# zju-vipa/ProtoPFormer

Measured on AMD Instinct MI355X. Metric: images/sec train step, deit_small+2000 protos, bs256, 1/2/4/8 MI355X, higher is better.
Workload: dtype bf16; 1 GPU; deit_small_patch16_224, synthetic 224x224, 2000x384 prototypes, 200 classes, k=81, batch 256/GPU (BASELINE.json configs[2]), train step = fwd+CE+PPC+bwd+allreduce+AdamW+EMA, DropPath 0.1; blocks after the token reservation run compacted on the 1+k reserved rows (equal to the masked full-length blocks to bf16 rounding); bf16 backbone: the reserved tokens differ from the fp32 reference's in ~2-3 % o; global_batch=256, parallelism=dp1

## Files before the change

### include/ppf_hip.h

```cpp
#ifndef PPF_HIP_H
#define PPF_HIP_H

#include <stddef.h>
#include <stdint.h>

#ifdef __cplusplus
extern "C" {
#endif

typedef struct ihipStream_t* ppf_stream_t;

#define PPF_ERR_SHAPE (-1)
#define PPF_ERR_ALIGN (-2)
#define PPF_ERR_ARG (-3)

#define PPF_ABI_VERSION 10

const char* ppf_last_error(void);
int ppf_abi_version(void);
int ppf_device_info(int* cu_count, int* clock_mhz, char* name, int name_len);
int ppf_stream_arm(ppf_stream_t stream, int on);
int ppf_stream_wait_stream(ppf_stream_t dst, ppf_stream_t src);
int64_t ppf_stream_mark(ppf_stream_t stream);
int ppf_stream_wait_mark(ppf_stream_t stream, int64_t ticket);
// ... 157 lines not shown
                        ppf_stream_t stream);
int ppf_assemble_tokens_bwd(const float* dx, void* dtok, float* dpos, float* dcls, int B, int Np, int D, int lead,
                            ppf_stream_t stream);
int ppf_sigmoid_bwd_blocks(int rows);
int ppf_sigmoid_bwd(const float* df, const float* f, void* dz, float* dbias, int rows, int cols, float* partial, size_t partial_bytes,
                    ppf_stream_t stream);
int ppf_adamw_step(float* p, const float* g, float* m, float* v, float* ema, void* p16, int64_t n, int nseg,
                   const int64_t* seg_bounds, const float* seg_lr, const float* seg_wd, float beta1, float beta2, float eps,
                   int step, float ema_decay, float grad_scale, ppf_stream_t stream);
int ppf_adamw_step_dev(float* p, const float* g, float* m, float* v, float* ema, void* p16, int64_t n, int nseg,
                       const int64_t* seg_bounds, const float* hyper, float beta1, float beta2, float eps, float ema_decay,
                       ppf_stream_t stream);
int ppf_adamw_step_guarded(float* p, const float* g, float* m, float* v, float* ema, void* p16, int64_t n, int nseg,
                           const int64_t* seg_bounds, const float* hyper, float beta1, float beta2, float eps, float ema_decay,
                           const float* loss, int* nonfinite_flag, ppf_stream_t stream);
int ppf_hyper_set(float* hyper, const float* host_vals, int n, ppf_stream_t stream);
int ppf_clip_grad_blocks(void);
int ppf_clip_grad_scale(const float* g, int64_t n, float max_norm, float pre_scale, float* partial, float* hyper, float* norm_out,
                        ppf_stream_t stream);
int ppf_droppath_scales(float* out, const float* keep, int nslot, int B, uint64_t seed, void* state_u64, ppf_stream_t stream);
int ppf_reserved_rows_map(const int* idx, int* rows, int B, int k, int N, ppf_stream_t stream);
int ppf_gather_rows(const void* src, const int* rows, void* dst, int nrows, int row_bytes, ppf_stream_t stream);
int ppf_scatter_rows(const void* src, const int* rows, void* dst, int nrows_src, int nrows_dst, int row_bytes, ppf_stream_t stream);
int ppf_memset_zero(void* ptr, size_t bytes, ppf_stream_t stream);
int ppf_copy_2d(void* dst, int64_t dst_pitch, const void* src, int64_t src_pitch, int64_t width, int64_t rows, ppf_stream_t stream);
int ppf_image_finish_u8(const void* in_u8_hwc, float* out_nchw, int B, int H, int W, const float* mean3, const float* std3,
                        const int* rects, uint64_t seed, const void* state_u64, ppf_stream_t stream);
#define PPF_MIX_KIND 0
#define PPF_MIX_YL 1
#define PPF_MIX_YH 2
// ... 27 lines not shown
```

### protopformer_amd/backbone.py

```python
import functools
import os

import torch
import torch.nn as nn

from . import _lib, ops
from .ops import EPI_ATOMIC, EPI_BF16, EPI_DGELU, EPI_F32, EPI_GELU, EPI_RESID, EPI_SIGMOID_F32

LN_EPS = 1e-6
_KEEP_CACHE = {}
_ROW_BWD_MAX_ELEMS = 12_000_000


def _row_bwd(M, D):
    return M * D <= _ROW_BWD_MAX_ELEMS


def droppath_scales(rates, B, device, training):
    slots = [r if training else 0.0 for r in rates]
    active = [i for i, r in enumerate(slots) if r > 0.0]
    if not active:
        return None, [-1] * len(slots)
    key = (tuple(slots), str(device))
    st = _KEEP_CACHE.get(key)
# ... 167 lines not shown
        d = ops.ew_bwd_f32(5, ops.linear_dgrad_f32(d, c.weight), x_in)
    ops.colsum_f32(d, gv(convs[0].bias))
    return ops.cast_bf16(d)


class WgradLane:

    def __init__(self, device):
        self.enabled = os.environ.get("PPF_WGRAD_STREAM", "1") != "0"
        self.streams = [torch.cuda.Stream(device=device)] if self.enabled else []
        self.raws = [st.cuda_stream for st in self.streams]
        self.last_read = {}
        self.tracked = set()
        self.held = []
        self.pending = []

    def track(self, t):
        self.tracked.add(t.data_ptr())
        return t

    def submit(self, fn, reads, tag=None, defer=False):
        if not self.enabled:
            fn()
            return
        self.pending.append((fn, reads, tag))
        self.held.extend(reads)
        if not defer:
            self.flush()

    def flush(self, tag=None):
        if not self.pending:
            return
        raw = self.raws[0]
        try:
            _lib.call("ppf_stream_wait_stream", raw, _lib.stream_ptr())
            for fn, reads, tg in self.pending:
                _lib.push_stream(raw)
                try:
                    fn()
                    ptrs = [t.data_ptr() for t in reads if t.data_ptr() in self.tracked]
                    if ptrs:
                        ticket = _lib.stream_mark(raw)
                        for q in ptrs:
                            self.last_read[q] = ticket
                finally:
                    _lib.pop_stream()
        finally:
            self.pending.clear()

    def before_overwrite(self, t):
# ... 2 lines not shown
        q = t.data_ptr()
        if any(r.data_ptr() == q for _, reads, _t in self.pending for r in reads):
            self.flush()
        ticket = self.last_read.pop(q, None)
        if ticket is not None:
            _lib.call("ppf_stream_wait_mark", _lib.stream_ptr(), ticket)

    def join(self):
        if self.enabled:
            self.flush()
            for raw in self.raws:
                _lib.call("ppf_stream_wait_stream", _lib.stream_ptr(), raw)
        self.last_read.clear()
        self.tracked.clear()
        self.held.clear()


def wgrad_lane(store):
    lane = getattr(store, "_wgrad_lane", None)
    if lane is None:
        lane = store._wgrad_lane = WgradLane(store.device)
    return lane


_ROLL_TAIL = 1
_ROLL_BATCH = 3


def _wgrad(store, dy16, x16, weight, bias=None, defer=False):
    gw = store.grad_view(weight)
# ... 105 lines not shown
        return None, bias_done
    prev, Lp = below
    dyb = next_dyb(dyb)
    norm_bwd(dqkv, qkv.weight, dn1, L["x"], L["mean1"], L["rstd1"], blk.norm1,
             branch_out(store, dyb, Lp["s2"], Nl, getattr(prev, "gamma_2", None), Lp["raw2"]), prev.mlp.fc2.bias)
    return dyb, not fused


def embed_bwd(ppnet, store, saved, dx, lead):
    feats = ppnet.features
    pe = feats.patch_embed
    Np, D = pe.num_patches, dx.shape[1]
    gv = store.grad_view
    dtok = ops.assemble_tokens_bwd(dx, gv(feats.pos_embed).reshape(Np + lead, D), gv(feats.cls_token).reshape(D) if lead else None,
                                   dx.shape[0] // (Np + lead), Np, D, lead)
    _wgrad(store, dtok, saved["cols"], pe.proj.weight, pe.proj.bias)
    lane = wgrad_lane(store)
    gs = getattr(ppnet, "_grad_sync", None)
    if gs is not None:
        chunk_ready(gs, lane, gs.head_chunk)
    lane.join()


def deit_backward(ppnet, store, saved, df):
    feats = ppnet.features
    layers, head = saved["layers"], saved["head"]
    x_last = saved["x_last"]
    B, N, D = x_last.shape
    M = B * N
    dev = x_last.device
    lane = wgrad_lane(store)
    lnb = functools.partial(ops.layernorm_bwd, lane=lane, defer_reduce=True)
# ... 12 lines not shown
                            attn_bwd=lambda blk, L, dao: ops.attn_bwd(L["qkv"], L["ao"], dao, L["rowmax"], L["zinv"], B, feats.num_heads, L["N"], D,
                                                                      policy=L["policy"], self_keep=True, eps_n=L["eps_n"]))
    bias_done = True
    for i in range(len(layers) - 1, -1, -1):
        L = layers[i]
        Nl = L["N"]
        row_tile = row_tile_bwd(store, feats.blocks[i], D, ops.rowgemm_tile_rows(B * Nl, Nl, backward=True)) if _row_bwd(B * Nl, D) else None
        dyb, bias_done = bwd(feats.blocks[i], store, L, dx, dyb, bias_done, (feats.blocks[i - 1], layers[i - 1]) if i > 0 else None,
                             row_tile=row_tile)
        if i > 0 and L["rows"] is not None:
            Mf = B * layers[i - 1]["N"]
            dx = ops.scatter_rows(dx, L["rows"], Mf)
            dyb = lane.track(ops.scatter_rows(dyb, L["rows"], Mf))
        if gs is not None and i in gs.block_chunk:
            chunk_ready(gs, lane, gs.block_chunk[i])
    if layers and layers[0]["rows"] is not None:
        dx = ops.scatter_rows(dx, layers[0]["rows"], B * (feats.patch_embed.num_patches + 1))
    embed_bwd(ppnet, store, saved, dx, 1)


class TokensFn(torch.autograd.Function):

    @staticmethod
    def forward(ctx, img, ppnet, dp, *params):
        store = ppnet.flat_store()
        store.refresh_bf16()
        feats = ppnet.features
        need_bwd = any(ctx.needs_input_grad)
        if need_bwd and "t16_params" in ppnet._arch_fns:
            if store._t16 is None:
# ... 34 lines not shown
```

### protopformer_amd/cait.py

```python
import functools
import os

import torch
import torch.nn as nn

from . import ops
from .backbone import (LN_EPS, _ROLL_BATCH, _dp, _wgrad, block_bwd, block_fwd, branch_out, chunk_ready, dyb_ring, embed_bwd, embed_tokens, head_bwd,
                       mlp_bwd, row_tile_bwd, row_tile_fwd, t16_params, wgrad_lane)
from .deit import _Mlp, _PatchEmbed, _init_vit
from .ops import EPI_ATOMIC, EPI_BF16, EPI_F32, EPI_GELU, EPI_RESID


class _TalkingHeadAttn(nn.Module):
    def __init__(self, dim, num_heads):
        super().__init__()
        self.num_heads = num_heads
        self.qkv = nn.Linear(dim, dim * 3, bias=True)
        self.proj = nn.Linear(dim, dim)
        self.proj_l = nn.Linear(num_heads, num_heads)
        self.proj_w = nn.Linear(num_heads, num_heads)


class _ClassAttn(nn.Module):
    def __init__(self, dim, num_heads):
# ... 230 lines not shown
    scratch = torch.empty((B, D), dtype=torch.bfloat16, device=dev)
    lnb(None, None, None, None, None, None, None, dres_in=dcls, cast_out=scratch, dbias_next=gv(feats.cls_token).reshape(D))
    dx = ops.copy_2d(torch.empty((B, N * D), dtype=torch.float32, device=dev), du2[:, D:]).reshape(M, D)
    dyb = lane.track(torch.empty((M, D), dtype=torch.bfloat16, device=dev))
    last = feats.blocks[-1]
    lnb(None, None, None, None, None, None, None, dres_in=dx, dbias_next=gv(last.mlp.fc2.bias),
        **branch_out(store, dyb, sa[-1]["s2"], N, last.gamma_2, sa[-1]["raw2"]))
    bwd = functools.partial(block_bwd, next_dyb=dyb_ring(lane, D), lnb=lnb, row_tile=row_tile_bwd(store, last, D, ops.rowgemm_tile_rows(M, N)),
                            dgrad=lambda dy16, weight, rows, which: ops.gemm(dy16, store.w16(weight), trans_b=True, epi=EPI_BF16),
                            attn_bwd=lambda blk, L, dao: _th_attention_bwd(store, blk, L, dao, B, H, N, D))
    bias_done = True
    for i in range(len(sa) - 1, -1, -1):
        dyb, bias_done = bwd(feats.blocks[i], store, sa[i], dx, dyb, bias_done, (feats.blocks[i - 1], sa[i - 1]) if i > 0 else None)
        if gs is not None and i in gs.block_chunk:
            chunk_ready(gs, lane, gs.block_chunk[i])
    embed_bwd(ppnet, store, saved, dx, 0)


CAIT_FNS = dict(embed=functools.partial(embed_tokens, lead=0), blocks=cait_blocks_fwd, backward=cait_backward, t16_params=t16_params)
```

### protopformer_amd/csrc/elementwise.hip

```cpp
#include "ppf_common.h"
#include "ppf_hip.h"

namespace {

__global__ __launch_bounds__(256) void cast_kernel(const float* __restrict__ in, bf16_t* __restrict__ out, int64_t n8) {
    for (int64_t i = (int64_t)blockIdx.x * 256 + threadIdx.x; i < n8; i += (int64_t)gridDim.x * 256) {
        const float4 a = reinterpret_cast<const float4*>(in)[2 * i], b = reinterpret_cast<const float4*>(in)[2 * i + 1];
        reinterpret_cast<uint4*>(out)[i] = make_uint4(pack_bf16x2(a.x, a.y), pack_bf16x2(a.z, a.w), pack_bf16x2(b.x, b.y), pack_bf16x2(b.z, b.w));
    }
}

__global__ __launch_bounds__(256) void widen_kernel(const bf16_t* __restrict__ in, float* __restrict__ out, int64_t n8) {
    for (int64_t i = (int64_t)blockIdx.x * 256 + threadIdx.x; i < n8; i += (int64_t)gridDim.x * 256) {
        const uint4 u = reinterpret_cast<const uint4*>(in)[i];
        const float2 a = unpack_bf16x2(u.x), b = unpack_bf16x2(u.y), c = unpack_bf16x2(u.z), d = unpack_bf16x2(u.w);
        reinterpret_cast<float4*>(out)[2 * i] = make_float4(a.x, a.y, b.x, b.y);
        reinterpret_cast<float4*>(out)[2 * i + 1] = make_float4(c.x, c.y, d.x, d.y);
    }
}

__global__ __launch_bounds__(256) void im2col_kernel(const float* __restrict__ img, bf16_t* __restrict__ cols, int B, int C,
                                                     int H, int W, int p, int64_t total8) {
    const int gh = H / p, gw = W / p, pp8 = p / 8, kdim = C * p * p;
    for (int64_t i = (int64_t)blockIdx.x * 256 + threadIdx.x; i < total8; i += (int64_t)gridDim.x * 256) {
// ... 53 lines not shown
        dp[0] += sx; dp[1] += sy;
        if (t < lead && dcls) { dcls[c] += sx; dcls[c + 1] += sy; }
    }
}

struct Seg { int64_t begin, end; float lr, wd; };
constexpr int MAX_SEGS = 8;
struct AdamParams {
    float* p; const float* g; float* m; float* v; float* ema; bf16_t* p16;
    int64_t n; int nseg; Seg seg[MAX_SEGS];
    float beta1, beta2, eps, bc1, bc2_sqrt, ema_decay, grad_scale;
    const float* hyper;
    const float* guard;
    int* nonfinite;
};
__global__ __launch_bounds__(256) void adamw_kernel(AdamParams a) {
    if (a.guard) {
        const float loss = *a.guard;
        if (!(fabsf(loss) <= 3.4028234e38f)) {
            if (blockIdx.x == 0 && threadIdx.x == 0) *a.nonfinite = 1;
            return;
        }
    }
    if (a.hyper) {
#pragma unroll
        for (int s = 0; s < MAX_SEGS; ++s) { a.seg[s].lr = a.hyper[s]; a.seg[s].wd = a.hyper[8 + s]; }
        a.bc1 = a.hyper[16]; a.bc2_sqrt = a.hyper[17]; a.grad_scale = a.hyper[18] * a.hyper[19];
    }
    const int64_t n4 = a.n / 4;
    for (int64_t i = (int64_t)blockIdx.x * 256 + threadIdx.x; i < n4; i += (int64_t)gridDim.x * 256) {
        const int64_t e0 = i * 4;
        float lr = 0.f, wd = 0.f;
#pragma unroll
        for (int s = 0; s < MAX_SEGS; ++s)
            if (s < a.nseg && e0 >= a.seg[s].begin && e0 < a.seg[s].end) { lr = a.seg[s].lr; wd = a.seg[s].wd; }
        float4 p = reinterpret_cast<float4*>(a.p)[i];
        const float4 g4 = reinterpret_cast<const float4*>(a.g)[i];
        float4 m = reinterpret_cast<float4*>(a.m)[i], v = reinterpret_cast<float4*>(a.v)[i];
        float pv[4] = {p.x, p.y, p.z, p.w}, gv[4] = {g4.x, g4.y, g4.z, g4.w}, mv[4] = {m.x, m.y, m.z, m.w}, vv[4] = {v.x, v.y, v.z, v.w};
#pragma unroll
        for (int k = 0; k < 4; ++k) {
            const float g = gv[k] * a.grad_scale;
            pv[k] *= (1.0f - lr * wd);
            mv[k] = a.beta1 * mv[k] + (1.0f - a.beta1) * g;
            vv[k] = a.beta2 * vv[k] + (1.0f - a.beta2) * g * g;
            const float denom = sqrtf(vv[k]) / a.bc2_sqrt + a.eps;
            pv[k] -= (lr / a.bc1) * (mv[k] / denom);
        }
        reinterpret_cast<float4*>(a.p)[i] = make_float4(pv[0], pv[1], pv[2], pv[3]);
        reinterpret_cast<float4*>(a.m)[i] = make_float4(mv[0], mv[1], mv[2], mv[3]);
        reinterpret_cast<float4*>(a.v)[i] = make_float4(vv[0], vv[1], vv[2], vv[3]);
        if (a.ema) {
            float4 e = reinterpret_cast<float4*>(a.ema)[i];
            const float d = a.ema_decay, o = 1.0f - a.ema_decay;
            reinterpret_cast<float4*>(a.ema)[i] = make_float4(e.x * d + o * pv[0], e.y * d + o * pv[1], e.z * d + o * pv[2], e.w * d + o * pv[3]);
        }
        if (a.p16) reinterpret_cast<uint2*>(a.p16)[i] = make_uint2(pack_bf16x2(pv[0], pv[1]), pack_bf16x2(pv[2], pv[3]));
    }
}

__global__ __launch_bounds__(256) void sigmoid_bwd_kernel(const float* __restrict__ df, const float* __restrict__ f, bf16_t* __restrict__ dz,
                                                          float* __restrict__ dbias, float* __restrict__ partial, int rows, int cols,
                                                          int rows_per_block) {
    const int r0 = blockIdx.x * rows_per_block, r1 = min(rows, r0 + rows_per_block);
    for (int c = threadIdx.x; c < cols; c += 256) {
        float acc = 0.f;
        for (int r = r0; r < r1; ++r) {
            const size_t o = (size_t)r * cols + c;
            const float fv = f[o];
            const bf16_t h = f32_to_bf16(df[o] * fv * (1.0f - fv));
// ... 164 lines not shown
    const int tc = (cols + 63) / 64, r0 = (b / tc) * 64, c0 = (b % tc) * 64;
    const int tx = threadIdx.x & 63, ty = threadIdx.x >> 6;
#pragma unroll
    for (int k = 0; k < 16; ++k) {
        const int r = r0 + ty + 4 * k, c = c0 + tx;
        tile[ty + 4 * k][tx] = (r < rows && c < cols) ? s[(size_t)r * cols + c] : (bf16_t)0;
    }
    __syncthreads();
#pragma unroll
    for (int k = 0; k < 16; ++k) {
        const int c = c0 + ty + 4 * k, r = r0 + tx;
        if (c < cols && r < rows) d[(size_t)c * rows + r] = tile[tx][ty + 4 * k];
    }
}

}

extern "C" {

int ppf_cast_f32_bf16(const float* in, void* out, int64_t n, hipStream_t stream) {
    PPF_CHECK_ARG(n > 0 && (n % 8) == 0, PPF_ERR_SHAPE, "ppf_cast_f32_bf16: n=%lld must be a positive multiple of 8", (long long)n);
    hipLaunchKernelGGL(cast_kernel, dim3(grid_for(n / 8)), dim3(256), 0, stream, in, (bf16_t*)out, n / 8);
    PPF_LAUNCH_CHECK();
    return 0;
}

int ppf_cast_bf16_f32(const void* in, float* out, int64_t n, hipStream_t stream) {
    PPF_CHECK_ARG(in && out && n > 0 && (n % 8) == 0, PPF_ERR_SHAPE, "ppf_cast_bf16_f32: n=%lld must be a positive multiple of 8", (long long)n);
    hipLaunchKernelGGL(widen_kernel, dim3(grid_for(n / 8)), dim3(256), 0, stream, (const bf16_t*)in, out, n / 8);
    PPF_LAUNCH_CHECK();
// ... 72 lines not shown
        a.seg[s].begin = seg_bounds[s]; a.seg[s].end = seg_bounds[s + 1];
    }
    a.beta1 = beta1; a.beta2 = beta2; a.eps = eps; a.bc1 = a.bc2_sqrt = 1.f; a.ema_decay = ema_decay; a.grad_scale = 1.f; a.hyper = hyper;
    a.guard = loss; a.nonfinite = nonfinite_flag;
    hipLaunchKernelGGL(adamw_kernel, dim3(grid_for(n / 4)), dim3(256), 0, stream, a);
    PPF_LAUNCH_CHECK();
    return 0;
}

int ppf_adamw_step_dev(float* p, const float* g, float* m, float* v, float* ema, void* p16, int64_t n, int nseg,
                       const int64_t* seg_bounds, const float* hyper, float beta1, float beta2, float eps, float ema_decay,
                       hipStream_t stream) {
    return ppf_adamw_step_guarded(p, g, m, v, ema, p16, n, nseg, seg_bounds, hyper, beta1, beta2, eps, ema_decay, nullptr, nullptr, stream);
}

int ppf_hyper_set(float* hyper, const float* host_vals, int n, hipStream_t stream) {
    PPF_CHECK_ARG(hyper && host_vals && n >= 1 && n <= 20, PPF_ERR_ARG, "ppf_hyper_set: bad arguments");
    HyperVals h;
    for (int i = 0; i < 20; ++i) h.v[i] = i < n ? host_vals[i] : 0.f;
    h.n = n;
    hipLaunchKernelGGL(hyper_set_kernel, dim3(1), dim3(64), 0, stream, hyper, h);
    PPF_LAUNCH_CHECK();
    return 0;
}

int ppf_clip_grad_blocks(void) { return 512; }

int ppf_clip_grad_scale(const float* g, int64_t n, float max_norm, float pre_scale, float* partial, float* hyper, float* norm_out,
                        hipStream_t stream) {
    PPF_CHECK_ARG(n > 0 && (n % 4) == 0 && max_norm > 0.f && partial && hyper, PPF_ERR_ARG, "ppf_clip_grad_scale: bad arguments");
// ... 89 lines not shown
```

### protopformer_amd/engine.py

```python
import math
import os
import sys

import torch
import torch.distributed as dist

from . import _lib, ops
from .protopformer import CrossEntropyLoss, WeightedLossFn

DEFAULT_LRS = {"features": 1e-4, "add_on_layers": 3e-3, "prototype_vectors": 3e-3}

_HY_LR, _HY_WD, _HY_BC1, _HY_BC2, _HY_GSCALE, _HY_CLIP, _HY_N = 0, 8, 16, 17, 18, 19, 20


def _unwrap(model):
    if isinstance(model, (torch.nn.parallel.DistributedDataParallel, torch.nn.DataParallel)):
        raise RuntimeError("protopformer_amd: do not wrap the model in DistributedDataParallel / DataParallel -- gradients are written into "
                           "a flat buffer by the HIP kernels and exchanged by engine.GradSync (pass grad_sync=make_grad_sync(model, optimizer))")
    return model


class FlatAdamW:
    def __init__(self, ppnet, joint_optimizer_lrs=None, weight_decay=0.05, betas=(0.9, 0.999), eps=1e-8, ema_decay=None):
        ppnet = _unwrap(ppnet)
        lrs = dict(DEFAULT_LRS if joint_optimizer_lrs is None else joint_optimizer_lrs)
        self.ppnet = ppnet
        self.store = ppnet.flat_store()
        st = self.store
        wds = {"features": 1e-3, "add_on_layers": 1e-3, "prototype_vectors": weight_decay, "prototype_vectors_global": weight_decay}
        lr_of = {"features": lrs["features"], "add_on_layers": lrs["add_on_layers"], "prototype_vectors": lrs["prototype_vectors"],
                 "prototype_vectors_global": lrs["prototype_vectors"]}
        self.betas, self.eps = betas, eps
        self.param_groups = []
        for n, b, e in st.segments:
# ... 33 lines not shown
            h[_HY_WD + i] = g["weight_decay"]
        h[_HY_BC1] = 1.0 - self.betas[0] ** self.step_count
        h[_HY_BC2] = math.sqrt(1.0 - self.betas[1] ** self.step_count)
        h[_HY_GSCALE] = float(self.grad_scale)
        n = _HY_CLIP if self._clip_issued else _HY_N
        self._clip_issued = False
        _lib.call("ppf_hyper_set", self._hyper, h.data_ptr(), n)

    def clip_grad_norm(self, max_norm):
        if self._clip_partial is None:
            self._clip_partial = torch.empty(_lib.lib().ppf_clip_grad_blocks(), dtype=torch.float32, device=self.store.device)
        _lib.call("ppf_clip_grad_scale", self.store.grads, self.store.total, float(max_norm), float(self.grad_scale), self._clip_partial,
                  self._hyper, self.grad_norm)
        self._clip_issued = True

    def launch_update(self, loss_guard=None):
        st = self.store
        _lib.call("ppf_adamw_step_guarded", st.params, st.grads, self.exp_avg, self.exp_avg_sq, self.ema, st.bf16, st.total, len(self.param_groups),
                  self._bounds.data_ptr(), self._hyper, self.betas[0], self.betas[1], self.eps, self.ema_decay,
                  loss_guard, self.nonfinite if loss_guard is not None else None)
        st.mark_bf16_written()

    def step(self, loss_guard=None):
        self._check_store()
        clip = self._clip_issued
        _lib.run_live(lambda: self._live_refresh(clip))
        self.launch_update(loss_guard)

    def _live_refresh(self, clip_issued):
        self._clip_issued = clip_issued
        self.refresh_hyper()

    def state_dict(self):
        state, groups, i = {}, [], 0
        for g in self.param_groups:
            ids = []
            for _, p, o, n in self.store.entries:
                if not (g["begin"] <= o < g["end"]):
                    continue
                if self.step_count > 0:
                    state[i] = dict(step=torch.tensor(float(self.step_count)), exp_avg=self.exp_avg[o:o + n].view(p.shape).clone(),
# ... 249 lines not shown

def chunk_plan(entries, total, cuts=None, n_chunks=None):
    block_offsets = [o for name, o in entries if name.startswith("features.blocks.") and name.split(".")[3] == "norm1" and name.endswith("weight")]
    depth = len(block_offsets)
    if cuts is None and n_chunks is not None:
        per = max(1, math.ceil(depth / max(1, n_chunks - 1)))
        cuts = list(range(per, depth, per))
    if cuts is None:
        cuts = readiness_cuts(depth)
    cuts = sorted({int(c) for c in cuts if 0 < int(c) < depth})
    norm_off = next(o for name, o in entries if name == "features.norm.weight")
    bounds = sorted({0, norm_off, total} | {block_offsets[c] for c in cuts})
    return bounds, {i: bounds.index(block_offsets[i]) for i in cuts}


def _forward_backward(model, criterion, samples, targets, optimizer, epoch, ppc_cov_coe, ppc_mean_coe, use_ppc_loss, grad_sync, check_finite,
                      max_norm):
    outputs, auxi = model(samples)
    loss = criterion(outputs, targets)
    cov = mean = None
    if use_ppc_loss:
        cov, mean = model.get_PPC_loss(auxi[2], auxi[3], auxi[4], targets)
        if epoch >= 20:
            loss = WeightedLossFn.apply(loss, cov, mean, ppc_cov_coe, ppc_mean_coe)
    if check_finite and not math.isfinite(loss.item()):
        print("Loss is {}, stopping training".format(loss.item()))
        sys.exit(1)
    optimizer.zero_grad()
    guard = loss.detach().reshape(1)
    if grad_sync is not None:
        box = [guard]
        _lib.run_live(lambda: box.__setitem__(0, grad_sync.reduce_guard(loss)))
        guard = box[0]
    model._grad_sync = grad_sync
    loss.backward(gradient=ops.const_scalar(loss.device, 1.0))
    model._grad_sync = None
    if grad_sync is not None:
        _lib.run_live(lambda: setattr(optimizer, "grad_scale", grad_sync.finish()))
    if max_norm is not None:
        optimizer.clip_grad_norm(max_norm)
    return loss, cov, mean, guard


def train_one_step(model, criterion, samples, targets, optimizer, epoch=20, ppc_cov_coe=0.1, ppc_mean_coe=0.5, use_ppc_loss=True,
                   grad_sync=None, check_finite=False, max_norm=None):
    _unwrap(model)
    loss, cov, mean, guard = _forward_backward(model, criterion, samples, targets, optimizer, epoch, ppc_cov_coe, ppc_mean_coe, use_ppc_loss,
                                               grad_sync, check_finite, max_norm)
    optimizer.step(loss_guard=guard)
    return loss.detach(), (cov.detach() if cov is not None else None), (mean.detach() if mean is not None else None)
# ... 21 lines not shown
        if want["ppc_branch"]:
            want.update(ppc_cov_coe=float(ppc_cov_coe), ppc_mean_coe=float(ppc_mean_coe))
            have.update(ppc_cov_coe=float(kw["ppc_cov_coe"]), ppc_mean_coe=float(kw["ppc_mean_coe"]))
        if want != have:
            raise RuntimeError(f"GraphedTrainStep was built for {have} but train_one_epoch(epoch={epoch}) needs {want}: "
                               "build a new GraphedTrainStep for this phase (the branch is baked into the captured graph)")

    def _capture(self, samples, targets):
        opt = self.optimizer
        self.static_in = (samples, targets) if self.adopt_inputs else (samples.clone(), targets.clone())
        if self.grad_sync is not None:
            opt.grad_scale = 1.0 / self.grad_sync.world
        torch.cuda.synchronize()
        self.graph = torch.cuda.CUDAGraph()
        with torch.cuda.graph(self.graph):
            loss, cov, mean, guard = _forward_backward(self.model, self.criterion, self.static_in[0], self.static_in[1], opt, **self.kw)
            opt.launch_update(guard)
            self.out = (loss.detach(), cov.detach() if cov is not None else None, mean.detach() if mean is not None else None)

    def __call__(self, samples, targets):
        opt = self.optimizer
        opt._check_store()
        self.calls += 1
        if self.graph is None:
            if self.calls <= self.warmup:
                return train_one_step(self.model, self.criterion, samples, targets, opt, **self.kw)
            self._capture(samples, targets)
        if samples.shape != self.static_in[0].shape or targets.shape != self.static_in[1].shape or samples.dtype != self.static_in[0].dtype:
            return train_one_step(self.model, self.criterion, samples, targets, opt, **self.kw)
        if samples.data_ptr() != self.static_in[0].data_ptr():
            self.static_in[0].copy_(samples, non_blocking=True)
        if targets.data_ptr() != self.static_in[1].data_ptr():
            self.static_in[1].copy_(targets, non_blocking=True)
        self._refresh_shadow()
        opt.refresh_hyper()
        self.graph.replay()
        return self.out

    def _refresh_shadow(self):
        st = self.optimizer.store
        if not st.bf16_fresh:
            st.refresh_bf16()


class ReplayedTrainStep(GraphedTrainStep):

    def __init__(self, *a, **kw):
        super().__init__(*a, **kw)
        self.rec = None

    def __call__(self, samples, targets):
        opt = self.optimizer
        opt._check_store()
        self.calls += 1
        if self.rec is None:
            if self.calls <= self.warmup:
                return train_one_step(self.model, self.criterion, samples, targets, opt, **self.kw)
# ... 151 lines not shown
```

### protopformer_amd/flat.py

```python
import torch

from . import ops

ALIGN = 8


class FlatStore:
    def __init__(self, module, groups):
        self.module = module
        self.entries = []
        self.segments = []
        off = 0
        for gname, plist in groups:
            begin = off
            for name, p in plist:
                if not p.requires_grad:
                    continue
                self.entries.append((name, p, off, p.numel()))
                off += (p.numel() + ALIGN - 1) // ALIGN * ALIGN
            self.segments.append((gname, begin, off))
        self.total = off
        dev = self.entries[0][1].device
        self.device = dev
        self.params = torch.zeros(off, dtype=torch.float32, device=dev)
        self.grads = torch.zeros(off, dtype=torch.float32, device=dev)
        self.bf16 = torch.zeros(off, dtype=torch.bfloat16, device=dev)
        self._views16 = {}
        self._gviews = {}
        with torch.no_grad():
            for name, p, o, n in self.entries:
                self.params[o:o + n].copy_(p.detach().reshape(-1))
                p.data = self.params[o:o + n].view(p.shape)
                self._views16[id(p)] = self.bf16[o:o + n].view(p.shape)
                self._gviews[id(p)] = self.grads[o:o + n].view(p.shape)
                p.grad = self._gviews[id(p)]
        self.bf16_fresh = False
        self._t16 = None

    def register_transposed(self, params):
        params = [p for p in params if id(p) in self._views16]
        if not params:
            return
        off, desc, tiles, views = 0, [], 0, {}
        by_id = {id(p): o for _, p, o, _ in self.entries}
        for p in params:
            rows, cols = p.shape[0], p.numel() // p.shape[0]
            desc.append((by_id[id(p)], off, rows, cols))
            tiles += ((rows + 63) // 64) * ((cols + 63) // 64)
            views[id(p)] = (off, rows, cols)
            off += (rows * cols + ALIGN - 1) // ALIGN * ALIGN
        buf = torch.empty(off, dtype=torch.bfloat16, device=self.device)
        self._t16 = dict(buf=buf, desc=torch.tensor(desc, dtype=torch.int64).to(self.device), n=len(desc), tiles=tiles, fresh=False,
                         views={k: buf[o:o + r * c].view(c, r) for k, (o, r, c) in views.items()})

    def refresh_t16(self):
        t = self._t16
        if t is not None and not t["fresh"]:
            ops.transpose_bf16_batched(self.bf16, t["buf"], t["desc"], t["n"], t["tiles"])
            t["fresh"] = True

    def w16t(self, p):
        return None if self._t16 is None else self._t16["views"].get(id(p))

    def refresh_bf16(self, force=False):
        if force or not self.bf16_fresh:
            ops.cast_bf16(self.params, self.bf16)
            self.bf16_fresh = True
            if self._t16 is not None:
                self._t16["fresh"] = False

    def w16(self, p):
        return self._views16[id(p)]

    def mark_bf16_written(self):
        self.bf16_fresh = True
        if self._t16 is not None:
            self._t16["fresh"] = False

    def invalidate(self):
        self.bf16_fresh = False
        if self._t16 is not None:
            self._t16["fresh"] = False

    def grad_view(self, p):
        g = self._gviews[id(p)]
        if p.grad is None or p.grad.data_ptr() != g.data_ptr():
            ops.zero_(g)
            p.grad = g
        return g

    def attach_all_grads(self):
        if all(p.grad is None for _, p, _, _ in self.entries):
# ... 16 lines not shown
```

Measured before the change: 17580 images/sec.

## Fuse AdamW with bf16 transpose via work-item table and optional early step

Adds a table-driven AdamW kernel that updates parameters tile by tile and writes both the bf16 copy and the transposed bf16 weights in one pass, so the separate batched transpose after the optimizer is no longer needed. It also adds an opt-in early step (PPF_EARLY_STEP) that launches the update for late-layer parameters during backward, once their gradients are final, to overlap it with the rest of backward. The fused path runs by default whenever transposed weights are registered. It costs a binary search per block and shared-memory tile staging, and adds complexity around stream ordering.

```diff
diff --git a/include/ppf_hip.h b/include/ppf_hip.h
--- a/include/ppf_hip.h
+++ b/include/ppf_hip.h
@@ -195,6 +195,10 @@
 int ppf_adamw_step_guarded(float* p, const float* g, float* m, float* v, float* ema, void* p16, int64_t n, int nseg,
                            const int64_t* seg_bounds, const float* hyper, float beta1, float beta2, float eps, float ema_decay,
                            const float* loss, int* nonfinite_flag, ppf_stream_t stream);
+int ppf_adamw_table_prepare(int64_t* table_host, int n_items, int64_t n, int64_t n_t);
+int ppf_adamw_step_table(float* p, const float* g, float* m, float* v, float* ema, void* p16, void* p16t, int64_t n, int64_t n_t,
+                         const int64_t* table_dev, const int64_t* table_host, int first_item, int n_items, int ngroups, const float* hyper,
+                         float beta1, float beta2, float eps, float ema_decay, const float* loss, int* nonfinite_flag, ppf_stream_t stream);
 int ppf_hyper_set(float* hyper, const float* host_vals, int n, ppf_stream_t stream);
 int ppf_clip_grad_blocks(void);
 int ppf_clip_grad_scale(const float* g, int64_t n, float max_norm, float pre_scale, float* partial, float* hyper, float* norm_out,
diff --git a/protopformer_amd/backbone.py b/protopformer_amd/backbone.py
--- a/protopformer_amd/backbone.py
+++ b/protopformer_amd/backbone.py
@@ -205,6 +205,7 @@
         self.tracked = set()
         self.held = []
         self.pending = []
+        self.main_first = []
 
     def track(self, t):
         self.tracked.add(t.data_ptr())
@@ -219,12 +220,18 @@
         if not defer:
             self.flush()
 
+    def on_flush(self, fn):
+        self.main_first.append(fn)
+
     def flush(self, tag=None):
         if not self.pending:
             return
         raw = self.raws[0]
         try:
             _lib.call("ppf_stream_wait_stream", raw, _lib.stream_ptr())
+            first, self.main_first = self.main_first, []
+            for fn in first:
+                fn()
             for fn, reads, tg in self.pending:
                 _lib.push_stream(raw)
                 try:
@@ -257,6 +264,7 @@
         self.last_read.clear()
         self.tracked.clear()
         self.held.clear()
+        self.main_first.clear()
 
 
 def wgrad_lane(store):
@@ -392,8 +400,13 @@
     gv = store.grad_view
     dtok = ops.assemble_tokens_bwd(dx, gv(feats.pos_embed).reshape(Np + lead, D), gv(feats.cls_token).reshape(D) if lead else None,
                                    dx.shape[0] // (Np + lead), Np, D, lead)
+    lane = wgrad_lane(store)
+    early = store.early_step
+    if early is not None and lane.enabled:
+        lane.on_flush(early.fire)
     _wgrad(store, dtok, saved["cols"], pe.proj.weight, pe.proj.bias)
-    lane = wgrad_lane(store)
+    if early is not None:
+        early.fire()
     gs = getattr(ppnet, "_grad_sync", None)
     if gs is not None:
         chunk_ready(gs, lane, gs.head_chunk)
@@ -436,6 +449,8 @@
             dyb = lane.track(ops.scatter_rows(dyb, L["rows"], Mf))
         if gs is not None and i in gs.block_chunk:
             chunk_ready(gs, lane, gs.block_chunk[i])
+        if store.early_step is not None and i == store.early_step.block:
+            store.early_step.mark(lane)
     if layers and layers[0]["rows"] is not None:
         dx = ops.scatter_rows(dx, layers[0]["rows"], B * (feats.patch_embed.num_patches + 1))
     embed_bwd(ppnet, store, saved, dx, 1)
diff --git a/protopformer_amd/cait.py b/protopformer_amd/cait.py
--- a/protopformer_amd/cait.py
+++ b/protopformer_amd/cait.py
@@ -268,6 +268,8 @@
         dyb, bias_done = bwd(feats.blocks[i], store, sa[i], dx, dyb, bias_done, (feats.blocks[i - 1], sa[i - 1]) if i > 0 else None)
         if gs is not None and i in gs.block_chunk:
             chunk_ready(gs, lane, gs.block_chunk[i])
+        if store.early_step is not None and i == store.early_step.block:
+            store.early_step.mark(lane)
     embed_bwd(ppnet, store, saved, dx, 0)
 
 
diff --git a/protopformer_amd/csrc/adamw_layout.h b/protopformer_amd/csrc/adamw_layout.h
--- /dev/null
+++ b/protopformer_amd/csrc/adamw_layout.h
@@ -0,0 +1,77 @@
+#pragma once
+#include <stdint.h>
+
+#if defined(__HIPCC__)
+#define PPF_AHD __host__ __device__ __forceinline__
+#else
+#define PPF_AHD inline
+#endif
+
+namespace ppfa {
+
+constexpr int TILE = 64;
+constexpr int RANGE_BLOCK = 4096;
+constexpr int ITEM_WORDS = 8;
+enum { IT_OFF = 0, IT_TOFF = 1, IT_ROWS = 2, IT_COLS = 3, IT_GROUP = 4, IT_BLK0 = 5, IT_NBLK = 6, IT_SPARE = 7 };
+constexpr int MAX_GROUPS = 8;
+
+PPF_AHD int64_t item_elems(const int64_t* it) { return it[IT_ROWS] > 0 ? it[IT_ROWS] * it[IT_COLS] : it[IT_COLS]; }
+
+PPF_AHD int64_t item_blocks(const int64_t* it) {
+    if (it[IT_ROWS] > 0) return ((it[IT_ROWS] + TILE - 1) / TILE) * ((it[IT_COLS] + TILE - 1) / TILE);
+    return (it[IT_COLS] + RANGE_BLOCK - 1) / RANGE_BLOCK;
+}
+
+inline int64_t adamw_table_prefix(int64_t* table, int n_items) {
+    int64_t b = 0;
+    for (int i = 0; i < n_items; ++i) {
+        int64_t* it = table + (int64_t)i * ITEM_WORDS;
+        it[IT_BLK0] = b;
+        it[IT_NBLK] = item_blocks(it);
+        b += it[IT_NBLK];
+    }
+    return b;
+}
+
+inline int adamw_table_check(const int64_t* table, int first, int n, int64_t n_flat, int64_t n_t, int* bad) {
+    for (int i = first; i < first + n; ++i) {
+        const int64_t* it = table + (int64_t)i * ITEM_WORDS;
+        *bad = i;
+        if (it[IT_GROUP] < 0 || it[IT_GROUP] >= MAX_GROUPS) return 1;
+        if (it[IT_ROWS] < 0 || it[IT_COLS] <= 0 || it[IT_ROWS] > INT32_MAX || it[IT_COLS] > INT32_MAX) return 2;
+        if (it[IT_OFF] < 0 || it[IT_OFF] % 4 != 0 || item_elems(it) > n_flat || it[IT_OFF] > n_flat - item_elems(it)) return 3;
+        if (it[IT_ROWS] == 0 && (it[IT_COLS] % 4 != 0 || it[IT_TOFF] != -1)) return 4;
+        if (it[IT_ROWS] > 0 && (it[IT_TOFF] < 0 || item_elems(it) > n_t || it[IT_TOFF] > n_t - item_elems(it))) return 5;
+        if (it[IT_NBLK] != item_blocks(it) || it[IT_BLK0] < 0) return 6;
+        const int64_t* pv = it - ITEM_WORDS;
+        if (i > first && it[IT_BLK0] != pv[IT_BLK0] + pv[IT_NBLK]) return 7;
+    }
+    return 0;
+}
+
+PPF_AHD int find_item(const int64_t* table, int first, int n, int64_t b) {
+    int lo = first, hi = first + n - 1;
+    while (lo < hi) {
+        const int mid = (lo + hi + 1) >> 1;
+        if (table[(int64_t)mid * ITEM_WORDS + IT_BLK0] <= b) lo = mid;
+        else hi = mid - 1;
+    }
+    return lo;
+}
+
+struct TilePos { int r0, c0; };
+PPF_AHD TilePos tile_pos(int64_t local, int cols) {
+    const int tc = (cols + TILE - 1) / TILE;
+    return {(int)(local / tc) * TILE, (int)(local % tc) * TILE};
+}
+
+PPF_AHD int64_t src_index(const int64_t* it, int r, int c) { return it[IT_OFF] + (int64_t)r * it[IT_COLS] + c; }
+PPF_AHD int64_t wt_index(const int64_t* it, int r, int c) { return it[IT_TOFF] + (int64_t)c * it[IT_ROWS] + r; }
+PPF_AHD int64_t range_begin(const int64_t* it, int64_t local) { return it[IT_OFF] + local * RANGE_BLOCK; }
+
+struct LanePos { int r, c; };
+PPF_AHD LanePos vec_lane(int t, int q) { return {(t >> 4) + 16 * q, 4 * (t & 15)}; }
+PPF_AHD LanePos scalar_lane(int t, int k) { return {(t >> 6) + 4 * k, t & 63}; }
+PPF_AHD LanePos wt_lane(int t, int k) { return {t & 63, (t >> 6) + 4 * k}; }
+
+}
diff --git a/protopformer_amd/csrc/elementwise.hip b/protopformer_amd/csrc/elementwise.hip
--- a/protopformer_amd/csrc/elementwise.hip
+++ b/protopformer_amd/csrc/elementwise.hip
@@ -1,5 +1,6 @@
 #include "ppf_common.h"
 #include "ppf_hip.h"
+#include "adamw_layout.h"
 
 namespace {
 
@@ -91,19 +92,35 @@
     const float* guard;
     int* nonfinite;
 };
-__global__ __launch_bounds__(256) void adamw_kernel(AdamParams a) {
-    if (a.guard) {
-        const float loss = *a.guard;
-        if (!(fabsf(loss) <= 3.4028234e38f)) {
-            if (blockIdx.x == 0 && threadIdx.x == 0) *a.nonfinite = 1;
-            return;
-        }
-    }
+__device__ __forceinline__ void adamw_update(float& p, float& m, float& v, const float g_in, const float lr, const float wd, const AdamParams& a) {
+    const float g = g_in * a.grad_scale;
+    p *= (1.0f - lr * wd);
+    m = a.beta1 * m + (1.0f - a.beta1) * g;
+    v = a.beta2 * v + (1.0f - a.beta2) * g * g;
+    const float denom = sqrtf(v) / a.bc2_sqrt + a.eps;
+    p -= (lr / a.bc1) * (m / denom);
+}
+__device__ __forceinline__ float ema_update(const float e, const float p, const AdamParams& a) {
+    const float d = a.ema_decay, o = 1.0f - a.ema_decay;
+    return __builtin_fmaf(e, d, o * p);
+}
+__device__ __forceinline__ bool adamw_skip(const AdamParams& a) {
+    if (!a.guard) return false;
+    const float loss = *a.guard;
+    if (fabsf(loss) <= 3.4028234e38f) return false;
+    if (blockIdx.x == 0 && threadIdx.x == 0) *a.nonfinite = 1;
+    return true;
+}
+__device__ __forceinline__ void adamw_load_hyper(AdamParams& a) {
     if (a.hyper) {
 #pragma unroll
         for (int s = 0; s < MAX_SEGS; ++s) { a.seg[s].lr = a.hyper[s]; a.seg[s].wd = a.hyper[8 + s]; }
         a.bc1 = a.hyper[16]; a.bc2_sqrt = a.hyper[17]; a.grad_scale = a.hyper[18] * a.hyper[19];
     }
+}
+__global__ __launch_bounds__(256) void adamw_kernel(AdamParams a) {
+    if (adamw_skip(a)) return;
+    adamw_load_hyper(a);
     const int64_t n4 = a.n / 4;
     for (int64_t i = (int64_t)blockIdx.x * 256 + threadIdx.x; i < n4; i += (int64_t)gridDim.x * 256) {
         const int64_t e0 = i * 4;
@@ -116,21 +133,13 @@
         float4 m = reinterpret_cast<float4*>(a.m)[i], v = reinterpret_cast<float4*>(a.v)[i];
         float pv[4] = {p.x, p.y, p.z, p.w}, gv[4] = {g4.x, g4.y, g4.z, g4.w}, mv[4] = {m.x, m.y, m.z, m.w}, vv[4] = {v.x, v.y, v.z, v.w};
 #pragma unroll
-        for (int k = 0; k < 4; ++k) {
-            const float g = gv[k] * a.grad_scale;
-            pv[k] *= (1.0f - lr * wd);
-            mv[k] = a.beta1 * mv[k] + (1.0f - a.beta1) * g;
-            vv[k] = a.beta2 * vv[k] + (1.0f - a.beta2) * g * g;
-            const float denom = sqrtf(vv[k]) / a.bc2_sqrt + a.eps;
-            pv[k] -= (lr / a.bc1) * (mv[k] / denom);
-        }
+        for (int k = 0; k < 4; ++k) adamw_update(pv[k], mv[k], vv[k], gv[k], lr, wd, a);
         reinterpret_cast<float4*>(a.p)[i] = make_float4(pv[0], pv[1], pv[2], pv[3]);
         reinterpret_cast<float4*>(a.m)[i] = make_float4(mv[0], mv[1], mv[2], mv[3]);
         reinterpret_cast<float4*>(a.v)[i] = make_float4(vv[0], vv[1], vv[2], vv[3]);
         if (a.ema) {
             float4 e = reinterpret_cast<float4*>(a.ema)[i];
-            const float d = a.ema_decay, o = 1.0f - a.ema_decay;
-            reinterpret_cast<float4*>(a.ema)[i] = make_float4(e.x * d + o * pv[0], e.y * d + o * pv[1], e.z * d + o * pv[2], e.w * d + o * pv[3]);
+            reinterpret_cast<float4*>(a.ema)[i] = make_float4(ema_update(e.x, pv[0], a), ema_update(e.y, pv[1], a), ema_update(e.z, pv[2], a), ema_update(e.w, pv[3], a));
         }
         if (a.p16) reinterpret_cast<uint2*>(a.p16)[i] = make_uint2(pack_bf16x2(pv[0], pv[1]), pack_bf16x2(pv[2], pv[3]));
     }
@@ -325,6 +334,106 @@
     }
 }
 
+struct AdamTableParams {
+    AdamParams a;
+    const int64_t* table;
+    int first, n_items;
+    int64_t blk_base;
+    bf16_t* wt;
+};
+
+template <int V>
+__device__ __forceinline__ void adamw_tile(const AdamParams& a, const int64_t* __restrict__ it, bf16_t* __restrict__ wt, bf16_t (*tile)[66],
+                                           const int64_t local, const float lr, const float wd) {
+    const int rows = (int)it[ppfa::IT_ROWS], cols = (int)it[ppfa::IT_COLS];
+    const ppfa::TilePos tp = ppfa::tile_pos(local, cols);
+    const int t = threadIdx.x;
+#pragma unroll
+    for (int q = 0; q < 16 / V; ++q) {
+        const ppfa::LanePos lp = V == 4 ? ppfa::vec_lane(t, q) : ppfa::scalar_lane(t, q);
+        const int r = tp.r0 + lp.r, c = tp.c0 + lp.c;
+        if (r >= rows || c >= cols) continue;
+        const int64_t e = ppfa::src_index(it, r, c);
+        float pv[V], gv[V], mv[V], vv[V];
+        if constexpr (V == 4) {
+            const float4 p = *reinterpret_cast<const float4*>(a.p + e), g = *reinterpret_cast<const float4*>(a.g + e);
+            const float4 m = *reinterpret_cast<const float4*>(a.m + e), v = *reinterpret_cast<const float4*>(a.v + e);
+            pv[0] = p.x; pv[1] = p.y; pv[2] = p.z; pv[3] = p.w; gv[0] = g.x; gv[1] = g.y; gv[2] = g.z; gv[3] = g.w;
+            mv[0] = m.x; mv[1] = m.y; mv[2] = m.z; mv[3] = m.w; vv[0] = v.x; vv[1] = v.y; vv[2] = v.z; vv[3] = v.w;
+        } else {
+            pv[0] = a.p[e]; gv[0] = a.g[e]; mv[0] = a.m[e]; vv[0] = a.v[e];
+        }
+#pragma unroll
+        for (int k = 0; k < V; ++k) adamw_update(pv[k], mv[k], vv[k], gv[k], lr, wd, a);
+        if constexpr (V == 4) {
+            *reinterpret_cast<float4*>(a.p + e) = make_float4(pv[0], pv[1], pv[2], pv[3]);
+            *reinterpret_cast<float4*>(a.m + e) = make_float4(mv[0], mv[1], mv[2], mv[3]);
+            *reinterpret_cast<float4*>(a.v + e) = make_float4(vv[0], vv[1], vv[2], vv[3]);
+            if (a.ema) {
+                const float4 x = *reinterpret_cast<const float4*>(a.ema + e);
+                *reinterpret_cast<float4*>(a.ema + e) = make_float4(ema_update(x.x, pv[0], a), ema_update(x.y, pv[1], a), ema_update(x.z, pv[2], a), ema_update(x.w, pv[3], a));
+            }
+            const uint32_t lo = pack_bf16x2(pv[0], pv[1]), hi = pack_bf16x2(pv[2], pv[3]);
+            *reinterpret_cast<uint2*>(a.p16 + e) = make_uint2(lo, hi);
+            uint32_t* tl = reinterpret_cast<uint32_t*>(&tile[lp.r][lp.c]);
+            tl[0] = lo; tl[1] = hi;
+        } else {
+            a.p[e] = pv[0]; a.m[e] = mv[0]; a.v[e] = vv[0];
+            if (a.ema) a.ema[e] = ema_update(a.ema[e], pv[0], a);
+            const bf16_t h = f32_to_bf16(pv[0]);
+            a.p16[e] = h;
+            tile[lp.r][lp.c] = h;
+        }
+    }
+    __syncthreads();
+#pragma unroll
+    for (int k = 0; k < 16; ++k) {
+        const ppfa::LanePos lp = ppfa::wt_lane(t, k);
+        const int r = tp.r0 + lp.r, c = tp.c0 + lp.c;
+        if (r < rows && c < cols) wt[ppfa::wt_index(it, r, c)] = tile[lp.r][lp.c];
+    }
+}
+
+__global__ __launch_bounds__(256) void adamw_table_kernel(AdamTableParams tp) {
+    __shared__ bf16_t tile[64][66];
+    AdamParams& a = tp.a;
+    if (adamw_skip(a)) return;
+    adamw_load_hyper(a);
+    const int64_t b = tp.blk_base + blockIdx.x;
+    const int64_t* __restrict__ it = tp.table + (int64_t)ppfa::find_item(tp.table, tp.first, tp.n_items, b) * ppfa::ITEM_WORDS;
+    const int64_t local = b - it[ppfa::IT_BLK0];
+    const int grp = (int)it[ppfa::IT_GROUP];
+    float lr = 0.f, wd = 0.f;
+#pragma unroll
+    for (int s = 0; s < MAX_SEGS; ++s)
+        if (s == grp) { lr = a.seg[s].lr; wd = a.seg[s].wd; }
+    if (it[ppfa::IT_ROWS] > 0) {
+        if ((it[ppfa::IT_COLS] & 3) == 0) adamw_tile<4>(a, it, tp.wt, tile, local, lr, wd);
+        else adamw_tile<1>(a, it, tp.wt, tile, local, lr, wd);
+        return;
+    }
+    const int64_t beg = ppfa::range_begin(it, local), end = it[ppfa::IT_OFF] + it[ppfa::IT_COLS];
+#pragma unroll
+    for (int q = 0; q < ppfa::RANGE_BLOCK / 1024; ++q) {
+        const int64_t e = beg + 4 * (int64_t)(threadIdx.x + 256 * q);
+        if (e >= end) break;
+        const int64_t i = e / 4;
+        const float4 p = reinterpret_cast<float4*>(a.p)[i], g4 = reinterpret_cast<const float4*>(a.g)[i];
+        const float4 m = reinterpret_cast<float4*>(a.m)[i], v = reinterpret_cast<float4*>(a.v)[i];
+        float pv[4] = {p.x, p.y, p.z, p.w}, gv[4] = {g4.x, g4.y, g4.z, g4.w}, mv[4] = {m.x, m.y, m.z, m.w}, vv[4] = {v.x, v.y, v.z, v.w};
+#pragma unroll
+        for (int k = 0; k < 4; ++k) adamw_update(pv[k], mv[k], vv[k], gv[k], lr, wd, a);
+        reinterpret_cast<float4*>(a.p)[i] = make_float4(pv[0], pv[1], pv[2], pv[3]);
+        reinterpret_cast<float4*>(a.m)[i] = make_float4(mv[0], mv[1], mv[2], mv[3]);
+        reinterpret_cast<float4*>(a.v)[i] = make_float4(vv[0], vv[1], vv[2], vv[3]);
+        if (a.ema) {
+            const float4 x = reinterpret_cast<float4*>(a.ema)[i];
+            reinterpret_cast<float4*>(a.ema)[i] = make_float4(ema_update(x.x, pv[0], a), ema_update(x.y, pv[1], a), ema_update(x.z, pv[2], a), ema_update(x.w, pv[3], a));
+        }
+        if (a.p16) reinterpret_cast<uint2*>(a.p16)[i] = make_uint2(pack_bf16x2(pv[0], pv[1]), pack_bf16x2(pv[2], pv[3]));
+    }
+}
+
 }
 
 extern "C" {
@@ -427,6 +536,45 @@
     return ppf_adamw_step_guarded(p, g, m, v, ema, p16, n, nseg, seg_bounds, hyper, beta1, beta2, eps, ema_decay, nullptr, nullptr, stream);
 }
 
+int ppf_adamw_table_prepare(int64_t* table_host, int n_items, int64_t n, int64_t n_t) {
+    PPF_CHECK_ARG(table_host && n_items > 0 && n > 0 && n_t >= 0, PPF_ERR_ARG, "ppf_adamw_table_prepare: bad arguments");
+    ppfa::adamw_table_prefix(table_host, n_items);
+    int bad = 0;
+    const int rule = ppfa::adamw_table_check(table_host, 0, n_items, n, n_t, &bad);
+    PPF_CHECK_ARG(rule == 0, PPF_ERR_ARG, "ppf_adamw_table_prepare: item %d breaks rule %d of adamw_table_check", bad, rule);
+    return 0;
+}
+
+int ppf_adamw_step_table(float* p, const float* g, float* m, float* v, float* ema, void* p16, void* p16t, int64_t n, int64_t n_t,
+                         const int64_t* table_dev, const int64_t* table_host, int first_item, int n_items, int ngroups, const float* hyper,
+                         float beta1, float beta2, float eps, float ema_decay, const float* loss, int* nonfinite_flag, hipStream_t stream) {
+    PPF_CHECK_ARG(p && g && m && v && p16 && n > 0 && ngroups >= 1 && ngroups <= MAX_SEGS && hyper && table_dev && table_host, PPF_ERR_ARG,
+                  "ppf_adamw_step_table: bad arguments");
+    PPF_CHECK_ARG(first_item >= 0 && n_items > 0, PPF_ERR_ARG, "ppf_adamw_step_table: empty item range");
+    PPF_CHECK_ARG((loss == nullptr) == (nonfinite_flag == nullptr), PPF_ERR_ARG, "ppf_adamw_step_table: loss and flag go together");
+    PPF_CHECK_ARG((((uintptr_t)p | (uintptr_t)g | (uintptr_t)m | (uintptr_t)v | (uintptr_t)ema) & 15) == 0 && (((uintptr_t)p16) & 7) == 0, PPF_ERR_ALIGN,
+                  "ppf_adamw_step_table: buffers must be 16-byte aligned");
+    int bad = 0;
+    const int rule = ppfa::adamw_table_check(table_host, first_item, n_items, n, p16t ? n_t : 0, &bad);
+    PPF_CHECK_ARG(rule == 0, PPF_ERR_ARG, "ppf_adamw_step_table: item %d breaks rule %d of adamw_table_check", bad, rule);
+    const int64_t* it0 = table_host + (int64_t)first_item * ppfa::ITEM_WORDS;
+    const int64_t* it1 = table_host + (int64_t)(first_item + n_items - 1) * ppfa::ITEM_WORDS;
+    const int64_t blocks = it1[ppfa::IT_BLK0] + it1[ppfa::IT_NBLK] - it0[ppfa::IT_BLK0];
+    PPF_CHECK_ARG(blocks > 0 && blocks < ((int64_t)1 << 31), PPF_ERR_ARG, "ppf_adamw_step_table: %lld workgroups", (long long)blocks);
+    for (int i = first_item; i < first_item + n_items; ++i)
+        PPF_CHECK_ARG(table_host[(int64_t)i * ppfa::ITEM_WORDS + ppfa::IT_GROUP] < ngroups, PPF_ERR_ARG, "ppf_adamw_step_table: item %d: group out of range", i);
+    AdamTableParams t;
+    AdamParams& a = t.a;
+    a.p = p; a.g = g; a.m = m; a.v = v; a.ema = ema; a.p16 = (bf16_t*)p16; a.n = n; a.nseg = ngroups;
+    for (int s = 0; s < MAX_SEGS; ++s) { a.seg[s].begin = a.seg[s].end = 0; a.seg[s].lr = a.seg[s].wd = 0.f; }
+    a.beta1 = beta1; a.beta2 = beta2; a.eps = eps; a.bc1 = a.bc2_sqrt = 1.f; a.ema_decay = ema_decay; a.grad_scale = 1.f; a.hyper = hyper;
+    a.guard = loss; a.nonfinite = nonfinite_flag;
+    t.table = table_dev; t.first = first_item; t.n_items = n_items; t.blk_base = it0[ppfa::IT_BLK0]; t.wt = (bf16_t*)p16t;
+    hipLaunchKernelGGL(adamw_table_kernel, dim3((unsigned)blocks), dim3(256), 0, stream, t);
+    PPF_LAUNCH_CHECK();
+    return 0;
+}
+
 int ppf_hyper_set(float* hyper, const float* host_vals, int n, hipStream_t stream) {
     PPF_CHECK_ARG(hyper && host_vals && n >= 1 && n <= 20, PPF_ERR_ARG, "ppf_hyper_set: bad arguments");
     HyperVals h;
diff --git a/protopformer_amd/engine.py b/protopformer_amd/engine.py
--- a/protopformer_amd/engine.py
+++ b/protopformer_amd/engine.py
@@ -18,6 +18,29 @@
         raise RuntimeError("protopformer_amd: do not wrap the model in DistributedDataParallel / DataParallel -- gradients are written into "
                            "a flat buffer by the HIP kernels and exchanged by engine.GradSync (pass grad_sync=make_grad_sync(model, optimizer))")
     return model
+
+
+class EarlyStep:
+
+    def __init__(self, opt, tab, guard):
+        self.opt, self.tab, self.guard, self.block = opt, tab, guard, tab["block"]
+        self.ready = self.fired = False
+        self.ticket = None
+
+    def mark(self, lane):
+        if lane.enabled:
+            lane.flush()
+            self.ticket = _lib.stream_mark(lane.raws[0])
+        self.ready = True
+
+    def fire(self):
+        if self.fired or not self.ready:
+            return
+        if self.ticket is not None:
+            _lib.call("ppf_stream_wait_mark", _lib.stream_ptr(), self.ticket)
+        tab = self.tab
+        self.opt._launch_table(tab, tab["n_late"], tab["n"] - tab["n_late"], self.guard)
+        self.fired = True
 
 
 class FlatAdamW:
@@ -81,17 +104,60 @@
                   self._hyper, self.grad_norm)
         self._clip_issued = True
 
+    def _work_table(self):
+        st = self.store
+        if st._t16 is None:
+            return None
+        if st.adamw_table is None:
+            cut, block = 0, None
+            try:
+                bounds, block_chunk = chunk_plan([(name, o) for name, _, o, _ in st.entries], st.total)
+                if block_chunk:
+                    cut, block = bounds[1], min(block_chunk)
+            except StopIteration:
+                pass
+            st.build_adamw_table(self._bounds.tolist(), cut)
+            st.adamw_table["block"] = block
+        return st.adamw_table
+
+    def _launch_table(self, tab, first, count, loss_guard):
+        st = self.store
+        _lib.call("ppf_adamw_step_table", st.params, st.grads, self.exp_avg, self.exp_avg_sq, self.ema, st.bf16, st._t16["buf"], st.total,
+                  st._t16["buf"].numel(), tab["dev"], tab["host"], first, count, len(self.param_groups), self._hyper, self.betas[0], self.betas[1],
+                  self.eps, self.ema_decay, loss_guard, self.nonfinite if loss_guard is not None else None)
+
+    def arm_early(self, loss_guard=None, refresh=True):
+        self._check_store()
+        tab = self._work_table()
+        if tab is None or tab["block"] is None or tab["n_late"] in (0, tab["n"]):
+            return False
+        if refresh:
+            clip = self._clip_issued
+            _lib.run_live(lambda: self._live_refresh(clip))
+        self.store.early_step = EarlyStep(self, tab, loss_guard)
+        return True
+
     def launch_update(self, loss_guard=None):
         st = self.store
-        _lib.call("ppf_adamw_step_guarded", st.params, st.grads, self.exp_avg, self.exp_avg_sq, self.ema, st.bf16, st.total, len(self.param_groups),
-                  self._bounds.data_ptr(), self._hyper, self.betas[0], self.betas[1], self.eps, self.ema_decay,
-                  loss_guard, self.nonfinite if loss_guard is not None else None)
-        st.mark_bf16_written()
+        early, st.early_step = st.early_step, None
+        tab = self._work_table()
+        if tab is None:
+            _lib.call("ppf_adamw_step_guarded", st.params, st.grads, self.exp_avg, self.exp_avg_sq, self.ema, st.bf16, st.total, len(self.param_groups),
+                      self._bounds.data_ptr(), self._hyper, self.betas[0], self.betas[1], self.eps, self.ema_decay,
+                      loss_guard, self.nonfinite if loss_guard is not None else None)
+            st.mark_bf16_written()
+            return
+        if early is not None and early.fired:
+            self._launch_table(tab, 0, tab["n_late"], loss_guard)
+        else:
+            self._launch_table(tab, 0, tab["n"], loss_guard)
+        st.mark_bf16_written(transposed=True)
 
     def step(self, loss_guard=None):
         self._check_store()
-        clip = self._clip_issued
-        _lib.run_live(lambda: self._live_refresh(clip))
+        if self.store.early_step is None:
+            clip = self._clip_issued
+            _lib.run_live(lambda: self._live_refresh(clip))
         self.launch_update(loss_guard)
 
     def _live_refresh(self, clip_issued):
@@ -371,8 +437,11 @@
     return bounds, {i: bounds.index(block_offsets[i]) for i in cuts}
 
 
+EARLY_STEP = os.environ.get("PPF_EARLY_STEP", "0") != "0"
+
+
 def _forward_backward(model, criterion, samples, targets, optimizer, epoch, ppc_cov_coe, ppc_mean_coe, use_ppc_loss, grad_sync, check_finite,
-                      max_norm):
+                      max_norm, arm_refresh=True):
     outputs, auxi = model(samples)
     loss = criterion(outputs, targets)
     cov = mean = None
@@ -390,7 +459,13 @@
         _lib.run_live(lambda: box.__setitem__(0, grad_sync.reduce_guard(loss)))
         guard = box[0]
     model._grad_sync = grad_sync
-    loss.backward(gradient=ops.const_scalar(loss.device, 1.0))
+    if EARLY_STEP and max_norm is None and (grad_sync is None or (grad_sync.world == 1 and not grad_sync.force)):
+        optimizer.arm_early(guard, refresh=arm_refresh)
+    try:
+        loss.backward(gradient=ops.const_scalar(loss.device, 1.0))
+    except BaseException:
+        optimizer.store.early_step = None
+        raise
     model._grad_sync = None
     if grad_sync is not None:
         _lib.run_live(lambda: setattr(optimizer, "grad_scale", grad_sync.finish()))
@@ -442,7 +517,8 @@
         torch.cuda.synchronize()
         self.graph = torch.cuda.CUDAGraph()
         with torch.cuda.graph(self.graph):
-            loss, cov, mean, guard = _forward_backward(self.model, self.criterion, self.static_in[0], self.static_in[1], opt, **self.kw)
+            loss, cov, mean, guard = _forward_backward(self.model, self.criterion, self.static_in[0], self.static_in[1], opt, arm_refresh=False,
+                                                       **self.kw)
             opt.launch_update(guard)
             self.out = (loss.detach(), cov.detach() if cov is not None else None, mean.detach() if mean is not None else None)
 
@@ -469,6 +545,7 @@
         st = self.optimizer.store
         if not st.bf16_fresh:
             st.refresh_bf16()
+        st.refresh_t16()
 
 
 class ReplayedTrainStep(GraphedTrainStep):
diff --git a/protopformer_amd/flat.py b/protopformer_amd/flat.py
--- a/protopformer_amd/flat.py
+++ b/protopformer_amd/flat.py
@@ -3,6 +3,28 @@
 from . import ops
 
 ALIGN = 8
+ITEM_WORDS = 8
+
+
+def adamw_work_items(total, matrices, group_bounds, cut):
+    up4 = lambda x: (x + 3) // 4 * 4
+    marks = {0, total, cut} | set(group_bounds)
+    for o, (_, r, c) in matrices.items():
+        marks |= {o, up4(o + r * c)}
+    marks = sorted(m for m in marks if 0 <= m <= total)
+    if any(m % 4 for m in marks):
+        raise ValueError("adamw_work_items: offsets, group bounds and the cut must be multiples of 4")
+    items = []
+    for a, b in zip(marks, marks[1:]):
+        grp = max(g for g in range(len(group_bounds) - 1) if group_bounds[g] <= a)
+        if a in matrices:
+            toff, r, c = matrices[a]
+            if b != up4(a + r * c):
+                raise ValueError(f"adamw_work_items: the matrix at {a} is cut by a bound at {b}")
+            items.append([a, toff, r, c, grp, 0, 0, 0])
+        else:
+            items.append([a, -1, 0, b - a, grp, 0, 0, 0])
+    return items, sum(1 for it in items if it[0] < cut)
 
 
 class FlatStore:
@@ -36,6 +58,8 @@
                 p.grad = self._gviews[id(p)]
         self.bf16_fresh = False
         self._t16 = None
+        self.adamw_table = None
+        self.early_step = None
 
     def register_transposed(self, params):
         params = [p for p in params if id(p) in self._views16]
@@ -51,6 +75,7 @@
             off += (rows * cols + ALIGN - 1) // ALIGN * ALIGN
         buf = torch.empty(off, dtype=torch.bfloat16, device=self.device)
         self._t16 = dict(buf=buf, desc=torch.tensor(desc, dtype=torch.int64).to(self.device), n=len(desc), tiles=tiles, fresh=False,
+                         items={o: (to, r, c) for o, to, r, c in desc},
                          views={k: buf[o:o + r * c].view(c, r) for k, (o, r, c) in views.items()})
 
     def refresh_t16(self):
@@ -58,6 +83,16 @@
         if t is not None and not t["fresh"]:
             ops.transpose_bf16_batched(self.bf16, t["buf"], t["desc"], t["n"], t["tiles"])
             t["fresh"] = True
+
+    def build_adamw_table(self, group_bounds, cut):
+        if self._t16 is None:
+            return None
+        items, n_late = adamw_work_items(self.total, self._t16["items"], list(group_bounds), cut)
+        host = torch.tensor(items, dtype=torch.int64).reshape(len(items), ITEM_WORDS).contiguous()
+        from . import _lib
+        _lib.call("ppf_adamw_table_prepare", host.data_ptr(), len(items), self.total, self._t16["buf"].numel())
+        self.adamw_table = dict(host=host, dev=host.to(self.device), n=len(items), n_late=n_late)
+        return self.adamw_table
 
     def w16t(self, p):
         return None if self._t16 is None else self._t16["views"].get(id(p))
@@ -72,10 +107,10 @@
     def w16(self, p):
         return self._views16[id(p)]
 
-    def mark_bf16_written(self):
+    def mark_bf16_written(self, transposed=False):
         self.bf16_fresh = True
         if self._t16 is not None:
-            self._t16["fresh"] = False
+            self._t16["fresh"] = bool(transposed)
 
     def invalidate(self):
         self.bf16_fresh = False
```

After: 17630 images/sec, median of 6. No clear change (+0.3%).
